# cmavro/GNN-RAG

Measured on NVIDIA H100. Metric: questions/sec (GNN forward+score) on WebQSP-shape subgraphs; agg-kernel HBM GB/s, higher is better.
Workload: dtype f32

## Files before the change

### gnn_rag_b200/csrc/linear_tc.cu

```cuda
#include "wgmma.cuh"

namespace gr {

int g_tc_cluster = 1;
int g_tc_bk = 32;
int g_tc_tma_store = 1;

namespace {

using namespace tc;
constexpr int kThreads = 384;
constexpr int kConsumerWarps = 8;
constexpr int kLaunchRegs = 168, kProducerRegs = 40, kConsumerRegs = 232;
static_assert(128 * kProducerRegs + 256 * kConsumerRegs <= kThreads * kLaunchRegs, "register budget");

__global__ void split_bf16_seg_kernel(const float* __restrict__ W, int64_t ldw, int64_t N, int64_t Kpad,
                                      int seg, int pitch, __nv_bfloat16* __restrict__ hi,
                                      __nv_bfloat16* __restrict__ lo, int64_t ldo) {
  const int64_t total = N * Kpad;
  const int64_t stride = (int64_t)gridDim.x * blockDim.x;
  for (int64_t i = (int64_t)blockIdx.x * blockDim.x + threadIdx.x; i < total; i += stride) {
    const int64_t n = i / Kpad, k = i - n * Kpad;
    const int sidx = (int)(k / pitch), c = (int)(k - (int64_t)sidx * pitch);
    float v = c < seg ? __ldg(W + n * ldw + (int64_t)sidx * seg + c) : 0.f;
    const __nv_bfloat16 h = __float2bfloat16_rn(v);
    hi[n * ldo + k] = h;
    lo[n * ldo + k] = __float2bfloat16_rn(v - __bfloat162float(h));
  }
}

__global__ void split_bf16_kernel(const float* __restrict__ A, int64_t lda, int64_t M, int64_t K,
                                  __nv_bfloat16* __restrict__ hi, __nv_bfloat16* __restrict__ lo,
                                  int64_t ldo, int vec_ok, int vec_st) {
  const int64_t kq = (K + 3) / 4;
  const int64_t total = M * kq;
  const int64_t stride = (int64_t)gridDim.x * blockDim.x;
  for (int64_t i = (int64_t)blockIdx.x * blockDim.x + threadIdx.x; i < total; i += stride) {
    const int64_t m = i / kq, k = (i - m * kq) * 4;
    float v[4] = {0.f, 0.f, 0.f, 0.f};
    const float* src = A + m * lda + k;
    if (vec_ok && k + 3 < K) {
      float4 t = __ldg(reinterpret_cast<const float4*>(src));
      v[0] = t.x; v[1] = t.y; v[2] = t.z; v[3] = t.w;
    } else {
#pragma unroll
      for (int q = 0; q < 4; ++q)
        if (k + q < K) v[q] = __ldg(src + q);
    }
    __nv_bfloat16 h[4], l[4];
#pragma unroll
    for (int q = 0; q < 4; ++q) {
      h[q] = __float2bfloat16_rn(v[q]);
      l[q] = __float2bfloat16_rn(v[q] - __bfloat162float(h[q]));
    }
    __nv_bfloat16* ph = hi + m * ldo + k;
    __nv_bfloat16* pl = lo + m * ldo + k;
    if (vec_st && k + 3 < ldo) {
      *reinterpret_cast<uint2*>(ph) = *reinterpret_cast<uint2*>(h);
      *reinterpret_cast<uint2*>(pl) = *reinterpret_cast<uint2*>(l);
    } else {
#pragma unroll
      for (int q = 0; q < 4; ++q)
        if (k + q < ldo) { ph[q] = h[q]; pl[q] = l[q]; }
    }
  }
}

struct TcParams {
  const float* bias;
  float* C;
  int64_t ldc;
  __nv_bfloat16* c_hi;
  __nv_bfloat16* c_lo;
  int64_t ldc16;
  const float* w_score;
  float* dots;
  int M, N, K, n_pad, n16, stages, num_tiles;
  uint32_t flags;
  int tma_store;
  int kg_T, kg_G, kg_pitch, kg_nkb, kg_one0, kg_one1, kg_nb0;
};

template <int NP, int CS, int BK, bool GROUPED>
__global__ void __launch_bounds__(kThreads, 1)
linear_tc_kernel(const __grid_constant__ CUtensorMap map_a_hi, const __grid_constant__ CUtensorMap map_a_lo,
                 const __grid_constant__ CUtensorMap map_w_hi, const __grid_constant__ CUtensorMap map_w_lo,
                 const __grid_constant__ CUtensorMap map_c, const __grid_constant__ CUtensorMap map_c_hi,
                 const __grid_constant__ CUtensorMap map_c_lo, const TcParams p) {
  extern __shared__ __align__(1024) uint8_t smem_raw[];
  uint8_t* smem = reinterpret_cast<uint8_t*>((reinterpret_cast<uintptr_t>(smem_raw) + 1023) & ~(uintptr_t)1023);
  const int a_bytes = BM * BK * 2;
  constexpr int w_bytes = NP * BK * 2;
  const bool single = (p.flags & GR_LINEAR_BF16_SINGLE) != 0;
  const int w_off = single ? a_bytes : 2 * a_bytes;
  const int stage_bytes = single ? a_bytes + w_bytes : 2 * a_bytes + 2 * w_bytes;
  uint8_t* s_out = smem + (size_t)p.stages * stage_bytes;
  uint64_t* bars = reinterpret_cast<uint64_t*>(s_out + 2 * kStageOutBytes);
  uint64_t* full_bar = bars;
  uint64_t* empty_bar = bars + p.stages;
  float* s_bias = reinterpret_cast<float*>(bars + 2 * p.stages);
  float* s_ws = s_bias + 256;
  for (int i = threadIdx.x; i < 256; i += kThreads) {
    s_bias[i] = (p.bias && i < p.N) ? p.bias[i] : 0.f;
    s_ws[i] = (p.w_score && i < p.N) ? p.w_score[i] : 0.f;
  }

  const int warp = threadIdx.x >> 5, lane = threadIdx.x & 31;
  const int nkb = GROUPED ? p.kg_nkb : (p.K + BK - 1) / BK;
  const int crank = CS > 1 ? (int)cluster_ctarank() : 0;
  const int ncluster = gridDim.x / CS, cid = blockIdx.x / CS;
  const int ngroups = (p.num_tiles + CS - 1) / CS;
  constexpr uint16_t kMask = (uint16_t)((1u << CS) - 1);

  if (threadIdx.x == 0) {
    for (int s = 0; s < p.stages; ++s) {
      mbar_init(&full_bar[s], 1);
      mbar_init(&empty_bar[s], kConsumerWarps * CS);
    }
    asm volatile("fence.mbarrier_init.release.cluster;" ::: "memory");
  }
  __syncthreads();
  if (CS > 1) cluster_sync_all();

  if (warp < 4) {
    asm volatile("setmaxnreg.dec.sync.aligned.u32 %0;" ::"n"(kProducerRegs));
    if (warp == 0 && lane == 0) {
      uint32_t phase = 0;
      int s = 0;
      constexpr int w_rows = NP / CS;
      const int w_slice = w_rows * BK * 2;
      for (int g = cid; g < ngroups; g += ncluster) {
        const int m0 = (g * CS + crank) * BM;
        for (int kb = 0; kb < nkb; ++kb) {
          mbar_wait(&empty_bar[s], phase ^ 1);
          uint8_t* st = smem + (size_t)s * stage_bytes;
          mbar_expect_tx(&full_bar[s], (uint32_t)stage_bytes);
          int a_col = kb * BK;
          if constexpr (GROUPED) {
            if (p.kg_nb0 == 0) {
              const int g = kb / p.kg_T, t = kb - g * p.kg_T, ni = p.kg_T >> 1;
              const int seg = t == 0 ? 0 : 1 + 2 * ((t - 1) % ni) + (t - 1) / ni;
              a_col = seg * p.kg_pitch + g * BK;
            } else {
              const int g = min(kb / p.kg_T, p.kg_G), t = kb - g * p.kg_T;
              a_col = t == 0 ? g * BK : p.kg_nb0 + (kb - g - 1) * BK;
            }
          }
          tma_load_2d(st, &map_a_hi, &full_bar[s], a_col, m0);
          if (!single) tma_load_2d(st + a_bytes, &map_a_lo, &full_bar[s], a_col, m0);
          if (CS == 1) {
            tma_load_2d(st + w_off, &map_w_hi, &full_bar[s], kb * BK, 0);
            if (!single) tma_load_2d(st + w_off + w_bytes, &map_w_lo, &full_bar[s], kb * BK, 0);
          } else {
            tma_load_2d_mc(st + w_off + crank * w_slice, &map_w_hi, &full_bar[s], kb * BK,
                           crank * w_rows, kMask);
            if (!single)
              tma_load_2d_mc(st + w_off + w_bytes + crank * w_slice, &map_w_lo, &full_bar[s], kb * BK,
                             crank * w_rows, kMask);
          }
          if (++s == p.stages) { s = 0; phase ^= 1; }
        }
      }
    }
  } else {
    asm volatile("setmaxnreg.inc.sync.aligned.u32 %0;" ::"n"(kConsumerRegs));
    const int cw = (warp - 4) >> 2, wq = warp & 3;
    const EpiOut e{s_bias, s_ws, (p.flags & GR_LINEAR_RELU) != 0};
    const int r = wq * 16 + (lane >> 2), cq = lane & 3;
    uint8_t* stg = s_out + (size_t)cw * kStageOutBytes;
    const bool issuer = wq == 0 && lane == 0;
    const bool vec_c = p.C && (p.ldc % 2 == 0) && ((reinterpret_cast<uintptr_t>(p.C) & 7) == 0);
    const bool vec_h = p.c_hi && (p.ldc16 % 2 == 0) && ((reinterpret_cast<uintptr_t>(p.c_hi) & 3) == 0) &&
                       ((reinterpret_cast<uintptr_t>(p.c_lo) & 3) == 0);
    uint32_t phase = 0;
    int s = 0;
    for (int g = cid; g < ngroups; g += ncluster) {
      const int tile = g * CS + crank;
      float acc[NP / 2];
#pragma unroll
      for (int i = 0; i < NP / 2; ++i) acc[i] = 0.f;
      int prev = -1;
      for (int kb = 0; kb < nkb; ++kb) {
        mbar_wait(&full_bar[s], phase);
        const uint32_t sa = smem_u32(smem + (size_t)s * stage_bytes);
        const uint32_t a_row = (uint32_t)(cw * WG_M * BK * 2);
        const uint64_t da_hi = make_smem_desc<BK>(sa + a_row), da_lo = make_smem_desc<BK>(sa + a_bytes + a_row);
        const uint64_t dw_hi = make_smem_desc<BK>(sa + w_off), dw_lo = make_smem_desc<BK>(sa + w_off + w_bytes);
        if constexpr (GROUPED) {
          if (kb >= p.kg_one0 && kb < p.kg_one1) mma_kblock<NP, BK, 1, false>(acc, da_hi, da_lo, dw_hi, dw_lo);
          else mma_kblock<NP, BK, BK / MMA_K, false>(acc, da_hi, da_lo, dw_hi, dw_lo);
        } else if (single) {
          mma_kblock<NP, BK, BK / MMA_K, true>(acc, da_hi, da_lo, dw_hi, dw_lo);
        } else {
          mma_kblock<NP, BK, BK / MMA_K, false>(acc, da_hi, da_lo, dw_hi, dw_lo);
        }
        wgmma_wait<1>();
        if (prev >= 0 && lane == 0) release_slot<CS>(&empty_bar[prev]);
        prev = s;
        if (++s == p.stages) { s = 0; phase ^= 1; }
      }
      wgmma_wait<0>();
      if (prev >= 0 && lane == 0) release_slot<CS>(&empty_bar[prev]);

      const int64_t row0 = (int64_t)tile * BM + cw * WG_M + r;
      float dot0 = 0.f, dot1 = 0.f;
#pragma unroll
      for (int q = 0; q < NP / 16; ++q) {
        const int c0 = 16 * q;
        if (c0 >= p.n_pad) continue;
        float v[8];
        epi_values(acc, q, cq, e, v, dot0, dot1);
        if (p.tma_store) {
          epi_store_tma(v, stg, r, cq, issuer, 1 + cw, &map_c, &map_c_hi, &map_c_lo, p.C != nullptr,
                        p.c_hi != nullptr, c0, tile * BM + cw * WG_M);
          continue;
        }
#pragma unroll
        for (int b = 0; b < 2; ++b) {
          const int col = c0 + 8 * b + 2 * cq;
#pragma unroll
          for (int hr = 0; hr < 2; ++hr) {
            const int64_t row = row0 + 8 * hr;
            if (row >= p.M) continue;
            const float x0 = v[4 * b + 2 * hr], x1 = v[4 * b + 2 * hr + 1];
            if (p.C) {
              float* c = p.C + row * p.ldc + col;
              if (vec_c && col + 1 < p.N) {
                *reinterpret_cast<float2*>(c) = make_float2(x0, x1);
              } else {
                if (col < p.N) c[0] = x0;
                if (col + 1 < p.N) c[1] = x1;
              }
            }
            if (p.c_hi) {
              uint32_t lo;
              const uint32_t hi = split_hi_lo(x0, x1, lo);
              unsigned short* ph = reinterpret_cast<unsigned short*>(p.c_hi + row * p.ldc16 + col);
              unsigned short* pl = reinterpret_cast<unsigned short*>(p.c_lo + row * p.ldc16 + col);
              if (vec_h && col + 1 < p.n16) {
                *reinterpret_cast<uint32_t*>(ph) = hi;
                *reinterpret_cast<uint32_t*>(pl) = lo;
              } else {
                if (col < p.n16) { ph[0] = (unsigned short)(hi & 0xFFFF); pl[0] = (unsigned short)(lo & 0xFFFF); }
                if (col + 1 < p.n16) { ph[1] = (unsigned short)(hi >> 16); pl[1] = (unsigned short)(lo >> 16); }
              }
            }
          }
        }
      }
      epi_dots(dot0, dot1, p.dots, row0, p.M, cq);
    }
    if (p.tma_store && issuer) asm volatile("cp.async.bulk.wait_group 0;" ::: "memory");
  }
  __syncthreads();
  if (CS > 1) cluster_sync_all();
}

struct TcPlan {
  int64_t kp;
  int n_pad, np, stages, bk;
  size_t a_plane_bytes, w_plane_bytes, total_bytes, w_only_bytes, smem_bytes;
  bool ok;
};

TcPlan plan_tc(int64_t M, int64_t N, int64_t K, bool single = false) {
  TcPlan t{};
  const int BK = g_tc_bk == 64 ? 64 : 32;
  t.ok = (N >= 8 && N <= 256 && K >= 8 && M >= 1);
  t.kp = (K + 7) / 8 * 8;
  t.n_pad = (int)((N + 15) / 16 * 16);
  t.np = t.n_pad <= 64 ? 64 : t.n_pad <= 128 ? 128 : t.n_pad <= 208 ? 208 : 256;
  const size_t stage = (single ? 1 : 2) * ((size_t)BM * BK * 2 + (size_t)t.np * BK * 2);
  int stages = (int)((227 * 1024 - 1024 - 2048 - 128 - 2 * kStageOutBytes) / stage);
  t.stages = stages > 8 ? 8 : stages;
  if (t.stages < 2) t.ok = false;
  t.bk = BK;
  t.smem_bytes = (size_t)t.stages * stage + 1024  + 2 * t.stages * 8 + 2 * 256 * 4 + 2 * kStageOutBytes;
  t.a_plane_bytes = align_up((size_t)M * t.kp * 2, 256);
  t.w_plane_bytes = align_up((size_t)N * t.kp * 2, 256);
  t.total_bytes = 2 * t.a_plane_bytes + 2 * t.w_plane_bytes;
  t.w_only_bytes = 2 * t.w_plane_bytes;
  return t;
}


int split_launch(const float* A, int64_t lda, int64_t M, int64_t K, __nv_bfloat16* hi, __nv_bfloat16* lo,
                 int64_t ldo, cudaStream_t stream) {
  int va = (lda % 4 == 0) && ((reinterpret_cast<uintptr_t>(A) & 15) == 0);
  int64_t work = M * ((K + 3) / 4);
  int grid = (int)std::min<int64_t>(ceil_div(work, 256), 32LL * sm_count());
  int vs = (ldo % 4 == 0) && ((reinterpret_cast<uintptr_t>(hi) & 7) == 0) &&
           ((reinterpret_cast<uintptr_t>(lo) & 7) == 0);
  split_bf16_kernel<<<grid, 256, 0, stream>>>(A, lda, M, K, hi, lo, ldo, va, vs);
  GR_CHECK_LAUNCH();
  return GR_OK;
}

template <int NP, int CS, int BK, bool GROUPED = false>
int launch_tc_cs(const CUtensorMap& m_a_hi, const CUtensorMap& m_a_lo, const CUtensorMap& m_w_hi,
                 const CUtensorMap& m_w_lo, const CUtensorMap& m_c, const CUtensorMap& m_c_hi,
                 const CUtensorMap& m_c_lo, const TcPlan& t, const TcParams& p, cudaStream_t stream) {
  const int ngroups = (p.num_tiles + CS - 1) / CS;
  const int nclusters = std::max(1, std::min(ngroups, sm_count() / CS));
  return launch_cluster<linear_tc_kernel<NP, CS, BK, GROUPED>>("gr_linear_tc", kLaunchRegs, CS, nclusters * CS, kThreads,
                                                               t.smem_bytes, stream, m_a_hi, m_a_lo, m_w_hi, m_w_lo,
                                                               m_c, m_c_hi, m_c_lo, p);
}

template <int NP>
int launch_tc_np(const CUtensorMap* const (&m)[7], int cs, const TcPlan& t, const TcParams& p, cudaStream_t stream) {
  if (p.kg_T) {
    if (cs == 2) return launch_tc_cs<NP, 2, 32, true>(*m[0], *m[1], *m[2], *m[3], *m[4], *m[5], *m[6], t, p, stream);
    return launch_tc_cs<NP, 1, 32, true>(*m[0], *m[1], *m[2], *m[3], *m[4], *m[5], *m[6], t, p, stream);
  }
  if (t.bk == 64) {
    if (cs == 2) return launch_tc_cs<NP, 2, 64>(*m[0], *m[1], *m[2], *m[3], *m[4], *m[5], *m[6], t, p, stream);
    return launch_tc_cs<NP, 1, 64>(*m[0], *m[1], *m[2], *m[3], *m[4], *m[5], *m[6], t, p, stream);
  }
  if (cs == 2) return launch_tc_cs<NP, 2, 32>(*m[0], *m[1], *m[2], *m[3], *m[4], *m[5], *m[6], t, p, stream);
  return launch_tc_cs<NP, 1, 32>(*m[0], *m[1], *m[2], *m[3], *m[4], *m[5], *m[6], t, p, stream);
}

int launch_tc(const __nv_bfloat16* a_hi, const __nv_bfloat16* a_lo, int64_t lda16,
              const __nv_bfloat16* w_hi, const __nv_bfloat16* w_lo, int64_t ldw16, const TcPlan& t,
              TcParams p, cudaStream_t stream) {
  p.n_pad = t.n_pad; p.stages = t.stages;
  p.num_tiles = (int)ceil_div(p.M, BM);
  int cs = (g_tc_cluster >= 2 && (t.np / 2) % 8 == 0 && p.num_tiles >= 2) ? 2 : 1;
  CUtensorMap m_a_hi, m_a_lo, m_w_hi, m_w_lo;
  const int64_t w_cols = p.kg_T ? ldw16 : p.K;
  const int64_t a_cols = p.kg_nb0 ? p.kg_nb0 + (int64_t)(p.kg_T - 1) * p.kg_pitch : p.K;
  if (!make_tmap(&m_a_hi, a_hi, p.M, a_cols, lda16, BM, t.bk) || !make_tmap(&m_a_lo, a_lo, p.M, a_cols, lda16, BM, t.bk) ||
      !make_tmap(&m_w_hi, w_hi, p.N, w_cols, ldw16, t.np / cs, t.bk) ||
      !make_tmap(&m_w_lo, w_lo, p.N, w_cols, ldw16, t.np / cs, t.bk)) {
    set_error("gr_linear_tc: cuTensorMapEncodeTiled failed (pointers must be 16-byte aligned, row strides "
              "multiples of 8 elements)");
    return GR_ERR_CUDA;
  }
  p.n16 = (int)std::min<int64_t>((p.N + 15) / 16 * 16, p.ldc16);
  CUtensorMap m_c, m_c_hi, m_c_lo;
  memset(&m_c, 0, sizeof(m_c)); memset(&m_c_hi, 0, sizeof(m_c_hi)); memset(&m_c_lo, 0, sizeof(m_c_lo));
  bool ok = g_tc_tma_store != 0;
  if (ok && p.C) ok = p.N % 4 == 0 && make_out_tmap(&m_c, p.C, p.M, p.N, p.ldc, 4);
  if (ok && p.c_hi) ok = make_out_tmap(&m_c_hi, p.c_hi, p.M, p.n16, p.ldc16, 2) &&
                         make_out_tmap(&m_c_lo, p.c_lo, p.M, p.n16, p.ldc16, 2);
  p.tma_store = ok ? 1 : 0;
  const CUtensorMap* m[7] = {&m_a_hi, &m_a_lo, &m_w_hi, &m_w_lo, &m_c, &m_c_hi, &m_c_lo};
  switch (t.np) {
    case 64: return launch_tc_np<64>(m, cs, t, p, stream);
    case 128: return launch_tc_np<128>(m, cs, t, p, stream);
    case 208: return launch_tc_np<208>(m, cs, t, p, stream);
    default: return launch_tc_np<256>(m, cs, t, p, stream);
  }
}

}

bool linear_tc_supported(int64_t M, int64_t N, int64_t K) {
  return plan_tc(M, N, K).ok && get_encode_fn() != nullptr;
}

}

extern "C" size_t gr_linear_tc_workspace_bytes(int64_t M, int64_t N, int64_t K) {
  if (M <= 0 || N <= 0 || K <= 0) return 0;
  return gr::plan_tc(M, N, K).total_bytes;
}

extern "C" size_t gr_linear_tc_planes_workspace_bytes(int64_t N, int64_t K) {
  if (N <= 0 || K <= 0) return 0;
  return gr::plan_tc(1, N, K).w_only_bytes;
}

extern "C" int gr_split_bf16(const float* A, int64_t lda, int64_t M, int64_t K, void* hi, void* lo,
                             int64_t ld_out, void* stream_) {
  using namespace gr;
  GR_CHECK_ARG(A && hi && lo, "null pointer");
  GR_CHECK_ARG(M > 0 && K > 0 && lda >= K && ld_out >= K && ld_out % 8 == 0, "bad shape / ld_out % 8 != 0");
  return split_launch(A, lda, M, K, reinterpret_cast<__nv_bfloat16*>(hi), reinterpret_cast<__nv_bfloat16*>(lo),
                      ld_out, reinterpret_cast<cudaStream_t>(stream_));
}

extern "C" int gr_linear_tc(const float* A, int64_t lda, const float* W, int64_t ldw, const float* bias,
                            float* C, int64_t ldc, int64_t M, int64_t N, int64_t K, uint32_t flags,
                            void* workspace, size_t workspace_bytes, void* stream_) {
  using namespace gr;
  cudaStream_t stream = reinterpret_cast<cudaStream_t>(stream_);
  GR_CHECK_ARG(A && W && C && workspace, "null pointer");
  GR_CHECK_ARG(M > 0 && N > 0 && K > 0, "M, N, K must be positive");
  GR_CHECK_ARG(lda >= K && ldw >= K && ldc >= N, "leading dimension smaller than row length");
  GR_CHECK_ARG(M < (int64_t)0x7fffffff - BM, "M exceeds int32 range");
  TcPlan t = plan_tc(M, N, K);
  if (!t.ok) {
    set_error("gr_linear_tc: unsupported shape M=%lld N=%lld K=%lld (need 8 <= N <= 256, K >= 8)",
              (long long)M, (long long)N, (long long)K);
    return GR_ERR_UNSUPPORTED;
  }
  if (int rc = check_workspace(__func__, workspace, workspace_bytes, t.total_bytes)) return rc;
  if ((reinterpret_cast<uintptr_t>(workspace) & 255) != 0) {
    set_error("gr_linear_tc: workspace must be 256-byte aligned");
    return GR_ERR_INVALID_ARG;
  }
  char* ws = reinterpret_cast<char*>(workspace);
  __nv_bfloat16* a_hi = reinterpret_cast<__nv_bfloat16*>(ws);
  __nv_bfloat16* a_lo = reinterpret_cast<__nv_bfloat16*>(ws + t.a_plane_bytes);
  __nv_bfloat16* w_hi = reinterpret_cast<__nv_bfloat16*>(ws + 2 * t.a_plane_bytes);
  __nv_bfloat16* w_lo = reinterpret_cast<__nv_bfloat16*>(ws + 2 * t.a_plane_bytes + t.w_plane_bytes);
  int rc = split_launch(A, lda, M, K, a_hi, a_lo, t.kp, stream);
  if (rc != GR_OK) return rc;
  rc = split_launch(W, ldw, N, K, w_hi, w_lo, t.kp, stream);
  if (rc != GR_OK) return rc;
  TcParams p{};
  p.bias = bias; p.C = C; p.ldc = ldc;
  p.M = (int)M; p.N = (int)N; p.K = (int)K; p.flags = flags;
  return launch_tc(a_hi, a_lo, t.kp, w_hi, w_lo, t.kp, t, p, stream);
}

extern "C" int gr_linear_tc_planes(const void* A_hi, const void* A_lo, int64_t lda16, const float* W,
                                   int64_t ldw, const float* bias, float* C, int64_t ldc, void* C_hi,
                                   void* C_lo, int64_t ldc16, const float* w_score, float* dots, int64_t M,
                                   int64_t N, int64_t K, int64_t k_seg, int64_t k_seg_pitch, uint32_t flags,
                                   void* workspace, size_t workspace_bytes, void* stream_) {
  using namespace gr;
  cudaStream_t stream = reinterpret_cast<cudaStream_t>(stream_);
  GR_CHECK_ARG(A_hi && (A_lo || (flags & GR_LINEAR_BF16_SINGLE)) && W && workspace, "null pointer");
  GR_CHECK_ARG(C || C_hi, "no output requested");
  GR_CHECK_ARG(M > 0 && N > 0 && K > 0, "M, N, K must be positive");
  const bool grouped = (flags & GR_LINEAR_K_GROUPED) != 0;
  const bool korder = (flags & GR_LINEAR_K_ORDER_PLANES) != 0;
  GR_CHECK_ARG(!korder || grouped, "GR_LINEAR_K_ORDER_PLANES modifies GR_LINEAR_K_GROUPED and needs it");
  if (grouped) {
    GR_CHECK_ARG(k_seg > 0 && k_seg_pitch >= k_seg && k_seg_pitch % 16 == 0,
                 "GR_LINEAR_K_GROUPED needs segmented K: k_seg > 0 and k_seg_pitch >= k_seg, a multiple of 16");
    GR_CHECK_ARG(K % k_seg_pitch == 0 && (K / k_seg_pitch) % 2 == 1,
                 "GR_LINEAR_K_GROUPED needs an odd number of segments (2 I + 1)");
    GR_CHECK_ARG(g_tc_bk != 64, "GR_LINEAR_K_GROUPED needs 32-column k-blocks (tc_bk = 32)");
    GR_CHECK_ARG(!(flags & GR_LINEAR_BF16_SINGLE), "GR_LINEAR_K_GROUPED does not combine with GR_LINEAR_BF16_SINGLE");
  }
  const bool segmented = grouped || (k_seg > 0 && k_seg_pitch > k_seg);
  GR_CHECK_ARG(lda16 >= K && lda16 % 8 == 0, "lda16 must be >= K and a multiple of 8");
  GR_CHECK_ARG(!segmented || K % k_seg_pitch == 0, "K must be a multiple of k_seg_pitch");
  GR_CHECK_ARG(ldw >= (segmented ? K / k_seg_pitch * k_seg : K), "ldw smaller than the weight row length");
  GR_CHECK_ARG(!C || ldc >= N, "ldc smaller than N");
  GR_CHECK_ARG(!C_hi || (C_lo && ldc16 >= N), "C_lo missing or ldc16 smaller than N");
  GR_CHECK_ARG(!dots || w_score, "dots requested without w_score");
  GR_CHECK_ARG(M < (int64_t)0x7fffffff - BM, "M exceeds int32 range");
  TcPlan t = plan_tc(M, N, K, (flags & GR_LINEAR_BF16_SINGLE) != 0);
  if (!t.ok) {
    set_error("gr_linear_tc_planes: unsupported shape M=%lld N=%lld K=%lld", (long long)M, (long long)N,
              (long long)K);
    return GR_ERR_UNSUPPORTED;
  }
  const int num_ins = grouped ? (int)(K / k_seg_pitch / 2) : 0;
  const GroupedK gk = grouped ? plan_grouped_k(k_seg_pitch, num_ins, N, korder) : GroupedK{};
// ... 46 lines not shown
```

### gnn_rag_b200/csrc/wgmma.cuh

```cuda
#pragma once
#include <cuda.h>
#include <cuda_bf16.h>

#include "common.cuh"

namespace gr {
namespace tc {

constexpr int BM = 128;
constexpr int WG_M = 64;
constexpr int MMA_K = 16;

struct GroupedK {
  int G, ksteps_last, nkb;
  int64_t kp;
  size_t w_plane_bytes;
};
GroupedK plan_grouped_k(int64_t pitch, int I, int64_t N_out, bool packed = false);
int grouped_w_split(const float* W, int64_t ldw, int64_t N_out, int D, int I, const GroupedK& k, __nv_bfloat16* hi,
                    __nv_bfloat16* lo, cudaStream_t stream);

typedef CUresult (*EncodeTiledFn)(CUtensorMap*, CUtensorMapDataType, cuuint32_t, void*, const cuuint64_t*,
                                  const cuuint64_t*, const cuuint32_t*, const cuuint32_t*,
                                  CUtensorMapInterleave, CUtensorMapSwizzle, CUtensorMapL2promotion,
                                  CUtensorMapFloatOOBfill);

inline EncodeTiledFn get_encode_fn() {
  static EncodeTiledFn fn = nullptr;
  static bool tried = false;
  if (!tried) {
    tried = true;
    void* p = nullptr;
    cudaDriverEntryPointQueryResult q;
    if (cudaGetDriverEntryPoint("cuTensorMapEncodeTiled", &p, cudaEnableDefault, &q) == cudaSuccess &&
        q == cudaDriverEntryPointSuccess)
      fn = reinterpret_cast<EncodeTiledFn>(p);
  }
  return fn;
}

inline bool make_tmap(CUtensorMap* m, const void* base, int64_t rows, int64_t cols, int64_t ld, int box_rows,
               int bk) {
  EncodeTiledFn fn = get_encode_fn();
  if (!fn) return false;
  cuuint64_t dims[2] = {(cuuint64_t)cols, (cuuint64_t)rows};
  cuuint64_t strides[1] = {(cuuint64_t)ld * 2};
  cuuint32_t box[2] = {(cuuint32_t)bk, (cuuint32_t)box_rows};
  cuuint32_t estr[2] = {1, 1};
  CUresult r = fn(m, CU_TENSOR_MAP_DATA_TYPE_BFLOAT16, 2, const_cast<void*>(base), dims, strides, box, estr,
                  CU_TENSOR_MAP_INTERLEAVE_NONE,
                  bk == 64 ? CU_TENSOR_MAP_SWIZZLE_128B : CU_TENSOR_MAP_SWIZZLE_64B,
                  CU_TENSOR_MAP_L2_PROMOTION_L2_256B, CU_TENSOR_MAP_FLOAT_OOB_FILL_NONE);
  return r == CUDA_SUCCESS;
}

inline bool make_out_tmap(CUtensorMap* m, const void* base, int64_t rows, int64_t cols, int64_t ld, int elem_bytes) {
  EncodeTiledFn fn = get_encode_fn();
  if (!fn) return false;
  if ((reinterpret_cast<uintptr_t>(base) & 15) != 0 || (ld * elem_bytes) % 16 != 0) return false;
  cuuint64_t dims[2] = {(cuuint64_t)cols, (cuuint64_t)rows};
  cuuint64_t strides[1] = {(cuuint64_t)ld * elem_bytes};
  cuuint32_t box[2] = {16u, (cuuint32_t)WG_M};
  cuuint32_t estr[2] = {1, 1};
  CUresult r = fn(m, elem_bytes == 4 ? CU_TENSOR_MAP_DATA_TYPE_FLOAT32 : CU_TENSOR_MAP_DATA_TYPE_BFLOAT16, 2,
                  const_cast<void*>(base), dims, strides, box, estr, CU_TENSOR_MAP_INTERLEAVE_NONE,
                  CU_TENSOR_MAP_SWIZZLE_NONE, CU_TENSOR_MAP_L2_PROMOTION_NONE,
                  CU_TENSOR_MAP_FLOAT_OOB_FILL_NONE);
  return r == CUDA_SUCCESS;
}

__device__ __forceinline__ uint32_t smem_u32(const void* p) {
  return (uint32_t)__cvta_generic_to_shared(p);
}
__device__ __forceinline__ void mbar_init(uint64_t* bar, uint32_t count) {
  asm volatile("mbarrier.init.shared::cta.b64 [%0], %1;" ::"r"(smem_u32(bar)), "r"(count));
}
__device__ __forceinline__ void mbar_expect_tx(uint64_t* bar, uint32_t bytes) {
  asm volatile("mbarrier.arrive.expect_tx.shared::cta.b64 _, [%0], %1;" ::"r"(smem_u32(bar)), "r"(bytes)
               : "memory");
}
__device__ __forceinline__ void mbar_wait(uint64_t* bar, uint32_t parity) {
  uint32_t ok = 0;
  while (!ok) {
    asm volatile(
        "{\n\t.reg .pred p;\n\t"
        "mbarrier.try_wait.parity.shared::cta.b64 p, [%1], %2;\n\t"
        "selp.u32 %0, 1, 0, p;\n\t}"
        : "=r"(ok)
        : "r"(smem_u32(bar)), "r"(parity)
        : "memory");
  }
}
__device__ __forceinline__ void mbar_arrive(uint64_t* bar) {
  asm volatile("mbarrier.arrive.shared::cta.b64 _, [%0];" ::"r"(smem_u32(bar)) : "memory");
}
__device__ __forceinline__ void mbar_arrive_cluster(uint64_t* bar, uint32_t rank) {
  uint32_t remote;
  asm volatile("mapa.shared::cluster.u32 %0, %1, %2;" : "=r"(remote) : "r"(smem_u32(bar)), "r"(rank));
  asm volatile("mbarrier.arrive.release.cluster.shared::cluster.b64 _, [%0];" ::"r"(remote) : "memory");
}
template <int CS>
__device__ __forceinline__ void release_slot(uint64_t* bar) {
  if (CS == 1) {
    mbar_arrive(bar);
  } else {
#pragma unroll
    for (int r = 0; r < CS; ++r) mbar_arrive_cluster(bar, (uint32_t)r);
  }
}
__device__ __forceinline__ void tma_load_2d(void* dst, const CUtensorMap* map, uint64_t* bar, int c0,
                                            int c1) {
  asm volatile(
      "cp.async.bulk.tensor.2d.shared::cluster.global.tile.mbarrier::complete_tx::bytes"
      " [%0], [%1, {%3, %4}], [%2];" ::"r"(smem_u32(dst)),
      "l"(reinterpret_cast<uint64_t>(map)), "r"(smem_u32(bar)), "r"(c0), "r"(c1)
      : "memory");
}
__device__ __forceinline__ void tma_load_2d_mc(void* dst, const CUtensorMap* map, uint64_t* bar, int c0,
                                               int c1, uint16_t mask) {
  asm volatile(
      "cp.async.bulk.tensor.2d.shared::cluster.global.tile.mbarrier::complete_tx::bytes.multicast::cluster"
      " [%0], [%1, {%4, %5}], [%2], %3;" ::"r"(smem_u32(dst)),
      "l"(reinterpret_cast<uint64_t>(map)), "r"(smem_u32(bar)), "h"(mask), "r"(c0), "r"(c1)
      : "memory");
}
__device__ __forceinline__ void tma_store_2d(const CUtensorMap* map, const void* src, int c0, int c1) {
  asm volatile("cp.async.bulk.tensor.2d.global.shared::cta.bulk_group [%0, {%2, %3}], [%1];" ::"l"(
                   reinterpret_cast<uint64_t>(map)),
               "r"(smem_u32(src)), "r"(c0), "r"(c1)
               : "memory");
}
__device__ __forceinline__ void named_bar_sync(int id, int nthreads) {
  asm volatile("bar.sync %0, %1;" ::"r"(id), "r"(nthreads) : "memory");
}
__device__ __forceinline__ void cluster_sync_all() {
  asm volatile("barrier.cluster.arrive.release.aligned;" ::: "memory");
  asm volatile("barrier.cluster.wait.acquire.aligned;" ::: "memory");
}
__device__ __forceinline__ uint32_t cluster_ctarank() {
  uint32_t r;
  asm volatile("mov.u32 %0, %%cluster_ctarank;" : "=r"(r));
  return r;
}

template <int BK>
__device__ __forceinline__ uint64_t make_smem_desc(uint32_t saddr) {
  uint64_t d = 0;
  d |= (uint64_t)((saddr >> 4) & 0x3FFF);
  d |= (uint64_t)1 << 16;
  d |= (uint64_t)((8 * BK * 2) >> 4) << 32;
  d |= (uint64_t)(BK == 64 ? 1 : 2) << 62;
  return d;
}

__device__ __forceinline__ void wgmma_fence() { asm volatile("wgmma.fence.sync.aligned;" ::: "memory"); }
__device__ __forceinline__ void wgmma_commit() { asm volatile("wgmma.commit_group.sync.aligned;" ::: "memory"); }
template <int N>
__device__ __forceinline__ void wgmma_wait() {
  asm volatile("wgmma.wait_group.sync.aligned %0;" ::"n"(N) : "memory");
}
template <int R>
__device__ __forceinline__ void acc_fence(float (&d)[R]) {
#pragma unroll
  for (int i = 0; i < R; ++i) asm volatile("" : "+f"(d[i])::"memory");
}

#define GR_ACC8(i) "+f"(d[OFF + (i)]), "+f"(d[OFF + (i) + 1]), "+f"(d[OFF + (i) + 2]), "+f"(d[OFF + (i) + 3]), \
                   "+f"(d[OFF + (i) + 4]), "+f"(d[OFF + (i) + 5]), "+f"(d[OFF + (i) + 6]), "+f"(d[OFF + (i) + 7])
#define GR_ACC32(i) GR_ACC8(i), GR_ACC8((i) + 8), GR_ACC8((i) + 16), GR_ACC8((i) + 24)
#define GR_REGS8 "%0, %1, %2, %3, %4, %5, %6, %7"
#define GR_REGS16 GR_REGS8 ", %8, %9, %10, %11, %12, %13, %14, %15"
#define GR_REGS32 GR_REGS16 ", %16, %17, %18, %19, %20, %21, %22, %23, %24, %25, %26, %27, %28, %29, %30, %31"
#define GR_REGS64 GR_REGS32 ", %32, %33, %34, %35, %36, %37, %38, %39, %40, %41, %42, %43, %44, %45, %46, %47, %48, " \
                  "%49, %50, %51, %52, %53, %54, %55, %56, %57, %58, %59, %60, %61, %62, %63"
#define GR_REGS104 GR_REGS64 ", %64, %65, %66, %67, %68, %69, %70, %71, %72, %73, %74, %75, %76, %77, %78, %79, " \
                   "%80, %81, %82, %83, %84, %85, %86, %87, %88, %89, %90, %91, %92, %93, %94, %95, %96, %97, %98, " \
                   "%99, %100, %101, %102, %103"
#define GR_REGS128 GR_REGS104 ", %104, %105, %106, %107, %108, %109, %110, %111, %112, %113, %114, %115, %116, " \
                   "%117, %118, %119, %120, %121, %122, %123, %124, %125, %126, %127"
#define GR_WGMMA(N, REGS, RA, RB, ...)                                                                   \
  asm volatile("{\n\t.reg .pred p;\n\tsetp.ne.b32 p, 1, 0;\n\t"                                          \
               "wgmma.mma_async.sync.aligned.m64n" #N "k16.f32.bf16.bf16 {" REGS "}, %" #RA ", %" #RB  \
               ", p, 1, 1, 0, 0;\n\t}"                                                                   \
               : __VA_ARGS__                                                                             \
               : "l"(a), "l"(b))
template <int N, int OFF, int R>
__device__ __forceinline__ void wgmma_bf16(float (&d)[R], uint64_t a, uint64_t b) {
  static_assert(OFF + N / 2 <= R, "accumulator range");
  if constexpr (N == 16) {
    GR_WGMMA(16, GR_REGS8, 8, 9, GR_ACC8(0));
// ... 47 lines not shown
}

struct EpiOut {
  const float* bias;
  const float* w_score;
  bool relu;
};

template <int R>
__device__ __forceinline__ void epi_values(const float (&a)[R], int q, int cq, const EpiOut& e, float (&v)[8],
                                           float& dot0, float& dot1) {
#pragma unroll
  for (int b = 0; b < 2; ++b) {
    const int col = 16 * q + 8 * b + 2 * cq;
    const float2 bb = *reinterpret_cast<const float2*>(e.bias + col);
    const float2 ww = *reinterpret_cast<const float2*>(e.w_score + col);
#pragma unroll
    for (int i = 0; i < 4; ++i) {
      float x = a[8 * q + 4 * b + i] + ((i & 1) ? bb.y : bb.x);
      if (e.relu) x = fmaxf(x, 0.f);
      v[4 * b + i] = x;
    }
    dot0 = fmaf(v[4 * b + 0], ww.x, dot0); dot0 = fmaf(v[4 * b + 1], ww.y, dot0);
    dot1 = fmaf(v[4 * b + 2], ww.x, dot1); dot1 = fmaf(v[4 * b + 3], ww.y, dot1);
  }
}

__device__ __forceinline__ uint32_t split_hi_lo(float x0, float x1, uint32_t& lo) {
  const __nv_bfloat162 h2 = __floats2bfloat162_rn(x0, x1);
  const float2 hf = __bfloat1622float2(h2);
  const __nv_bfloat162 l2 = __floats2bfloat162_rn(x0 - hf.x, x1 - hf.y);
  lo = *reinterpret_cast<const uint32_t*>(&l2);
  return *reinterpret_cast<const uint32_t*>(&h2);
}

constexpr int kStageOutBytes = WG_M * 16 * 4 + 2 * WG_M * 16 * 2;
__device__ __forceinline__ void epi_store_tma(const float (&v)[8], uint8_t* stg, int r, int cq, bool issuer,
                                              int bar_id, const CUtensorMap* map_c, const CUtensorMap* map_hi,
                                              const CUtensorMap* map_lo, bool has_c, bool has_planes, int c0, int m0) {
  if (issuer) asm volatile("cp.async.bulk.wait_group.read 0;" ::: "memory");
  named_bar_sync(bar_id, 128);
  float* s_c = reinterpret_cast<float*>(stg);
  uint32_t* s_h = reinterpret_cast<uint32_t*>(stg + WG_M * 16 * 4);
  uint32_t* s_l = reinterpret_cast<uint32_t*>(stg + WG_M * 16 * 4 + WG_M * 16 * 2);
#pragma unroll
  for (int b = 0; b < 2; ++b) {
    const int col = 8 * b + 2 * cq;
#pragma unroll
    for (int hr = 0; hr < 2; ++hr) {
      const int row = r + 8 * hr;
      const float x0 = v[4 * b + 2 * hr], x1 = v[4 * b + 2 * hr + 1];
      if (has_c) *reinterpret_cast<float2*>(s_c + row * 16 + col) = make_float2(x0, x1);
      if (has_planes) {
        uint32_t lo;
        const uint32_t hi = split_hi_lo(x0, x1, lo);
        s_h[row * 8 + col / 2] = hi;
        s_l[row * 8 + col / 2] = lo;
      }
    }
  }
  asm volatile("fence.proxy.async.shared::cta;" ::: "memory");
  named_bar_sync(bar_id, 128);
  if (issuer) {
    if (has_c) tma_store_2d(map_c, stg, c0, m0);
    if (has_planes) {
      tma_store_2d(map_hi, stg + WG_M * 16 * 4, c0, m0);
      tma_store_2d(map_lo, stg + WG_M * 16 * 4 + WG_M * 16 * 2, c0, m0);
    }
    asm volatile("cp.async.bulk.commit_group;" ::: "memory");
  }
}

__device__ __forceinline__ void epi_dots(float dot0, float dot1, float* dots, int64_t row0, int64_t M, int cq) {
  dot0 += __shfl_xor_sync(0xffffffffu, dot0, 1);
  dot0 += __shfl_xor_sync(0xffffffffu, dot0, 2);
  dot1 += __shfl_xor_sync(0xffffffffu, dot1, 1);
  dot1 += __shfl_xor_sync(0xffffffffu, dot1, 2);
  if (dots && cq == 0) {
    if (row0 < M) { dots[row0] = dot0; dots[M + row0] = 0.f; }
    if (row0 + 8 < M) { dots[row0 + 8] = dot1; dots[M + row0 + 8] = 0.f; }
  }
}

template <auto Kernel, typename... Args>
int launch_cluster(const char* fn, int launch_regs, int cs, int grid, int threads, size_t smem, cudaStream_t stream,
                   const Args&... args) {
  if (int rc = opt_in_smem<Kernel>(fn, 227 * 1024)) return rc;
  static int num_regs = 0;
  if (num_regs == 0) {
    cudaFuncAttributes fa{};
    GR_CHECK_CUDA_AS(fn, cudaFuncGetAttributes(&fa, Kernel));
    num_regs = fa.numRegs;
  }
  if (num_regs != launch_regs) {
    set_error("%s: kernel was compiled with %d registers per thread, the warpgroup budget needs %d", fn, num_regs,
              launch_regs);
    return GR_ERR_UNSUPPORTED;
  }
  cudaLaunchConfig_t cfg{};
  cfg.gridDim = dim3((unsigned)grid);
  cfg.blockDim = dim3((unsigned)threads);
  cfg.dynamicSmemBytes = smem;
  cfg.stream = stream;
  cudaLaunchAttribute attr[1];
  attr[0].id = cudaLaunchAttributeClusterDimension;
  attr[0].val.clusterDim.x = cs;
  attr[0].val.clusterDim.y = 1;
  attr[0].val.clusterDim.z = 1;
  cfg.attrs = attr;
  cfg.numAttrs = 1;
  GR_CHECK_CUDA_AS(fn, cudaLaunchKernelEx(&cfg, Kernel, args...));
  return GR_OK;
}

}
}
```

### include/gnnrag_b200.h

```cpp
#ifndef GNNRAG_B200_H_
#define GNNRAG_B200_H_

#include <stddef.h>
#include <stdint.h>

#ifdef __cplusplus
extern "C" {
#endif

#define GR_ABI_VERSION 1

typedef enum gr_status {
  GR_OK = 0,
  GR_ERR_INVALID_ARG = -1,
  GR_ERR_CUDA = -2,
  GR_ERR_WORKSPACE = -3,
  GR_ERR_UNSUPPORTED = -4
} gr_status;

#define GR_LINEAR_RELU 1u
#define GR_LINEAR_EXACT_FP32 2u
#define GR_LINEAR_BF16_SINGLE 8u
#define GR_LINEAR_W_PRESPLIT 4u

#define GR_LINEAR_K_GROUPED 16u
#define GR_LINEAR_K_ORDER_PLANES 32u

int gr_abi_version(void);
const char* gr_last_error(void);
int gr_set_option(const char* name, int64_t value);
static inline int64_t gr_pad4(int64_t n) { return (n + 3) & ~(int64_t)3; }

size_t gr_csr_build_workspace_bytes(int64_t F, int64_t Nt);
int gr_csr_build(const void* heads, const void* rels, const void* tails, int idx_bytes,
                 int64_t F, int64_t Nt, int64_t num_rel_rows,
                 int32_t* rowptr_t, int32_t* src_t, int32_t* rel_t, int32_t* fact_t,
                 int32_t* rowptr_h, int32_t* src_h, int32_t* rel_h, int32_t* fact_h,
                 int32_t* status, const int32_t* nfacts, void* workspace, size_t workspace_bytes, void* stream);

int gr_gather_f32(const float* in, const int32_t* fact, float* out, int64_t F, void* stream);

int gr_linear(const float* A, int64_t lda, const float* W, int64_t ldw, const float* bias,
              const float* addend, int64_t ld_addend, int64_t addend_rows,
              float* C, int64_t ldc, int64_t M, int64_t N, int64_t K, uint32_t flags, void* stream);

size_t gr_linear_tc_workspace_bytes(int64_t M, int64_t N, int64_t K);
int gr_linear_tc(const float* A, int64_t lda, const float* W, int64_t ldw, const float* bias,
                 float* C, int64_t ldc, int64_t M, int64_t N, int64_t K, uint32_t flags,
                 void* workspace, size_t workspace_bytes, void* stream);
size_t gr_linear_tc_planes_workspace_bytes(int64_t N, int64_t K);
int gr_linear_tc_planes(const void* A_hi, const void* A_lo, int64_t lda16, const float* W, int64_t ldw,
                        const float* bias, float* C, int64_t ldc, void* C_hi, void* C_lo, int64_t ldc16,
                        const float* w_score, float* dots, int64_t M, int64_t N, int64_t K,
                        int64_t k_seg, int64_t k_seg_pitch,
                        uint32_t flags, void* workspace, size_t workspace_bytes, void* stream);
int gr_split_bf16(const float* A, int64_t lda, int64_t M, int64_t K, void* hi, void* lo, int64_t ld_out,
                  void* stream);

int gr_aggregate(const int32_t* rowptr, const int32_t* src, const int32_t* rel, const float* w,
                 const float* prior, const float* table, const float* ins,
                 float* out, int64_t out_row_stride, int64_t out_col0, int64_t seg_stride,
                 float* possible, int B, int N, int D, int I, int64_t F, void* stream);

int gr_aggregate_backward(const int32_t* rowptr, const int32_t* src, const int32_t* rel, const float* w,
                          const float* prior, const float* table, const float* ins, const float* grad_out,
                          int64_t grad_row_stride, int64_t grad_col0, int64_t seg_stride, float* grad_table,
                          float* grad_ins, float* grad_prior, int B, int N, int D, int I, int64_t F, void* stream);

int gr_aggregate_dual(const int32_t* rowptr_t, const int32_t* src_t, const int32_t* rel_t,
                      const float* w_t, const int32_t* rowptr_h, const int32_t* src_h,
                      const int32_t* rel_h, const float* w_h, const float* prior,
                      const float* table_fwd, const float* table_inv, const float* ins,
                      float* out, int64_t out_row_stride, int64_t out_col0, int64_t seg_pitch,
                      void* out_hi, void* out_lo, int64_t ld_planes,
                      int B, int N, int D, int I, int64_t F, void* stream);

int gr_pad_table256(const float* table, int64_t ldt, int64_t rows, int D, float* pn, void* stream);
int gr_aggregate_dual_abs_supported(int N, int D, int64_t seg_pitch, int64_t R1);
int gr_aggregate_dual_abs(const int32_t* rowptr_t, const int32_t* src_t, const int32_t* rel_t, const float* w_t,
                         const int32_t* rowptr_h, const int32_t* src_h, const int32_t* rel_h, const float* w_h,
                         const float* prior, const float* pn_fwd, const float* pn_inv, int64_t table_rows,
                         const float* ins, void* out_hi, void* out_lo, int64_t ld_planes, int64_t out_col0,
                         int64_t seg_pitch, int B, int N, int D, int I, int64_t F, int32_t* tile_counter, void* stream);
#define GR_AGG_K_ORDER 1u
int gr_aggregate_dual_abs_ex(const int32_t* rowptr_t, const int32_t* src_t, const int32_t* rel_t, const float* w_t,
                             const int32_t* rowptr_h, const int32_t* src_h, const int32_t* rel_h, const float* w_h,
                             const float* prior, const float* pn_fwd, const float* pn_inv, int64_t table_rows,
                             const float* ins, void* out_hi, void* out_lo, int64_t ld_planes, int64_t out_col0,
                             int64_t seg_pitch, int B, int N, int D, int I, int64_t F, int32_t* tile_counter,
                             uint32_t flags, void* stream);

int gr_fused_profile_read(unsigned long long* out, int n);
int gr_fused_layer_supported(int64_t N_nodes, int64_t D, int64_t seg_pitch, int I, int64_t N_out);
size_t gr_fused_layer_workspace_bytes(int64_t D, int64_t seg_pitch, int I, int64_t N_out);
size_t gr_fused_ell_bytes(int B, int N_nodes, int64_t F);
int gr_fused_ell_build(const int32_t* rowptr_t, const int32_t* src_t, const int32_t* rel_t, const float* w_t,
                       const int32_t* rowptr_h, const int32_t* src_h, const int32_t* rel_h, const float* w_h,
                       int B, int N_nodes, int64_t F, void* ell, size_t ell_bytes, void* stream);
int gr_fused_layer(const int32_t* rowptr_t, const int32_t* src_t, const int32_t* rel_t, const float* w_t,
                   const int32_t* rowptr_h, const int32_t* src_h, const int32_t* rel_h, const float* w_h,
                   const float* prior, const float* pn_fwd, const float* pn_inv, const float* ins,
                   const void* h_hi, const void* h_lo, int64_t ldh16, int64_t seg_pitch, const float* W,
                   int64_t ldw, const float* bias, float* C, int64_t ldc, void* C_hi, void* C_lo,
                   int64_t ldc16, const float* w_score, float* dots, int B, int N_nodes, int D, int I,
                   int64_t N_out, int64_t F, uint32_t flags, void* workspace, size_t workspace_bytes,
                   void* ell, size_t ell_bytes, void* stream);

int gr_debug_store_probe(void* hi, void* lo, int64_t Nt, int64_t ld, int col_start, int ncols, int mode,
                         void* stream);

int gr_type_layer(const int32_t* rowptr_t, const int32_t* rel_t, const float* w_t,
                  const int32_t* rowptr_h, const int32_t* rel_h, const float* w_h,
                  const float* table, float* out, int64_t out_row_stride,
                  void* out_hi, void* out_lo, int64_t ld_planes,
                  int B, int N, int D, int64_t F, void* stream);

size_t gr_graft_stage_workspace_bytes(int64_t B, int64_t max_fact);
int gr_graft_stage(const int64_t* e2f_b, const int64_t* e2f_f, const int64_t* e2f_e, int64_t F_e2f,
                   const int64_t* f2e_b, const int64_t* f2e_e, const int64_t* f2e_f, int64_t F_f2e,
                   const int64_t* kb_fact_rel, int B, int N, int64_t max_fact, int64_t R1, int32_t* heads,
                   int32_t* rels, int32_t* tails, int32_t* slot_of, int32_t* nfacts, int32_t* status,
                   const int32_t* live, void* workspace, size_t workspace_bytes, void* stream);
int gr_graft_attention(const float* qh, const float* qmask, int Q, const float* rel, int64_t ldr, int64_t R1,
                       const int64_t* kb_fact_rel, int B, int64_t max_fact, int D, const int32_t* rowptr_h,
                       const int32_t* fact_h, const int32_t* slot_of, int N, float* W, float* Wt, float* E,
                       int32_t* status, void* stream);
int gr_graft_aggregate(const int32_t* rowptr_t, const int32_t* src_t, const int32_t* rel_t, const int32_t* fact_t,
                       const int32_t* slot_of, const float* Wt, const float* E, const float* prior,
                       const float* self_tab, int64_t ld_self, const float* head_tab, int64_t ld_head,
                       const float* q2e, double lambda, float* sum_out, int64_t ld_sum, void* out_hi, void* out_lo,
                       int64_t ld_planes, int64_t col_sum, int64_t col_indeg, int64_t col_q2e, float* indeg_out,
                       float* prior_next, int B, int N, int D, void* stream);

int gr_graft_dropout_mask(const int64_t* seed, double p, int64_t S, int D, uint8_t* mask, void* stream);
int gr_graft_aggregate_train(const int32_t* rowptr_t, const int32_t* src_t, const int32_t* rel_t,
                             const int32_t* fact_t, const int32_t* slot_of, const float* s, const float* self_tab,
                             int64_t ld_self, const float* head_tab, int64_t ld_head, const int64_t* seed, double p,
                             float* sum_out, int64_t ld_sum, int B, int N, int D, void* stream);
// ... 258 lines not shown
```

Measured before the change: 12890.

## Auto-select 2-CTA clusters and size persistent grid by occupancy query

Result: faster. 13060, median of 6 (+1.3%).

```diff
diff --git a/gnn_rag_b200/csrc/linear_tc.cu b/gnn_rag_b200/csrc/linear_tc.cu
--- a/gnn_rag_b200/csrc/linear_tc.cu
+++ b/gnn_rag_b200/csrc/linear_tc.cu
@@ -2,9 +2,23 @@
 
 namespace gr {
 
-int g_tc_cluster = 1;
+int g_tc_cluster = 0;
 int g_tc_bk = 32;
 int g_tc_tma_store = 1;
+
+int tc_cluster_grid(int64_t num_tiles, int cs, int max_active_clusters) {
+  const int64_t ngroups = (num_tiles + cs - 1) / cs;
+  return (int)std::max<int64_t>(1, std::min<int64_t>(ngroups, max_active_clusters));
+}
+
+int tc_cluster_size(int np, int64_t num_tiles, bool k_order) {
+  const bool pair_ok = (np / 2) % 8 == 0 && num_tiles >= 2;
+  if (g_tc_cluster == 1 || !pair_ok) return 1;
+  if (g_tc_cluster >= 2) return 2;
+  return k_order && np == 208 && num_tiles >= 4 * (int64_t)sm_count() ? 2 : 1;
+}
+
+int g_tc_last_launch[3] = {0, 0, 0};
 
 namespace {
 
@@ -131,10 +145,15 @@
       const int w_slice = w_rows * BK * 2;
       for (int g = cid; g < ngroups; g += ncluster) {
         const int m0 = (g * CS + crank) * BM;
+#ifdef GR_LINEAR_TC_DIAG_W_FIRST_TILE
+        const bool load_w = g == cid;
+#else
+        constexpr bool load_w = true;
+#endif
         for (int kb = 0; kb < nkb; ++kb) {
           mbar_wait(&empty_bar[s], phase ^ 1);
           uint8_t* st = smem + (size_t)s * stage_bytes;
-          mbar_expect_tx(&full_bar[s], (uint32_t)stage_bytes);
+          mbar_expect_tx(&full_bar[s], (uint32_t)(load_w ? stage_bytes : w_off));
           int a_col = kb * BK;
           if constexpr (GROUPED) {
             if (p.kg_nb0 == 0) {
@@ -148,10 +167,10 @@
           }
           tma_load_2d(st, &map_a_hi, &full_bar[s], a_col, m0);
           if (!single) tma_load_2d(st + a_bytes, &map_a_lo, &full_bar[s], a_col, m0);
-          if (CS == 1) {
+          if (load_w && CS == 1) {
             tma_load_2d(st + w_off, &map_w_hi, &full_bar[s], kb * BK, 0);
             if (!single) tma_load_2d(st + w_off + w_bytes, &map_w_lo, &full_bar[s], kb * BK, 0);
-          } else {
+          } else if (load_w) {
             tma_load_2d_mc(st + w_off + crank * w_slice, &map_w_hi, &full_bar[s], kb * BK,
                            crank * w_rows, kMask);
             if (!single)
@@ -195,12 +214,12 @@
           mma_kblock<NP, BK, BK / MMA_K, false>(acc, da_hi, da_lo, dw_hi, dw_lo);
         }
         wgmma_wait<1>();
-        if (prev >= 0 && lane == 0) release_slot<CS>(&empty_bar[prev]);
+        if (prev >= 0 && lane == 0) release_slot<CS, false>(&empty_bar[prev]);
         prev = s;
         if (++s == p.stages) { s = 0; phase ^= 1; }
       }
       wgmma_wait<0>();
-      if (prev >= 0 && lane == 0) release_slot<CS>(&empty_bar[prev]);
+      if (prev >= 0 && lane == 0) release_slot<CS, false>(&empty_bar[prev]);
 
       const int64_t row0 = (int64_t)tile * BM + cw * WG_M + r;
       float dot0 = 0.f, dot1 = 0.f;
@@ -300,11 +319,13 @@
 int launch_tc_cs(const CUtensorMap& m_a_hi, const CUtensorMap& m_a_lo, const CUtensorMap& m_w_hi,
                  const CUtensorMap& m_w_lo, const CUtensorMap& m_c, const CUtensorMap& m_c_hi,
                  const CUtensorMap& m_c_lo, const TcPlan& t, const TcParams& p, cudaStream_t stream) {
-  const int ngroups = (p.num_tiles + CS - 1) / CS;
-  const int nclusters = std::max(1, std::min(ngroups, sm_count() / CS));
-  return launch_cluster<linear_tc_kernel<NP, CS, BK, GROUPED>>("gr_linear_tc", kLaunchRegs, CS, nclusters * CS, kThreads,
-                                                               t.smem_bytes, stream, m_a_hi, m_a_lo, m_w_hi, m_w_lo,
-                                                               m_c, m_c_hi, m_c_lo, p);
+  constexpr auto kernel = linear_tc_kernel<NP, CS, BK, GROUPED>;
+  int max_active = 0;
+  if (int rc = max_active_clusters<kernel>("gr_linear_tc", CS, kThreads, t.smem_bytes, &max_active)) return rc;
+  const int nclusters = tc_cluster_grid(p.num_tiles, CS, max_active);
+  g_tc_last_launch[0] = CS; g_tc_last_launch[1] = nclusters; g_tc_last_launch[2] = max_active;
+  return launch_cluster<kernel>("gr_linear_tc", kLaunchRegs, CS, nclusters * CS, kThreads, t.smem_bytes, stream,
+                                m_a_hi, m_a_lo, m_w_hi, m_w_lo, m_c, m_c_hi, m_c_lo, p);
 }
 
 template <int NP>
@@ -326,7 +347,7 @@
               TcParams p, cudaStream_t stream) {
   p.n_pad = t.n_pad; p.stages = t.stages;
   p.num_tiles = (int)ceil_div(p.M, BM);
-  int cs = (g_tc_cluster >= 2 && (t.np / 2) % 8 == 0 && p.num_tiles >= 2) ? 2 : 1;
+  const int cs = tc_cluster_size(t.np, p.num_tiles, p.kg_nb0 > 0);
   CUtensorMap m_a_hi, m_a_lo, m_w_hi, m_w_lo;
   const int64_t w_cols = p.kg_T ? ldw16 : p.K;
   const int64_t a_cols = p.kg_nb0 ? p.kg_nb0 + (int64_t)(p.kg_T - 1) * p.kg_pitch : p.K;
@@ -370,6 +391,18 @@
 extern "C" size_t gr_linear_tc_planes_workspace_bytes(int64_t N, int64_t K) {
   if (N <= 0 || K <= 0) return 0;
   return gr::plan_tc(1, N, K).w_only_bytes;
+}
+
+extern "C" int gr_linear_tc_cluster_grid(int64_t num_tiles, int cluster, int max_active_clusters) {
+  if (num_tiles < 1 || cluster < 1 || max_active_clusters < 1) return 0;
+  return gr::tc_cluster_grid(num_tiles, cluster, max_active_clusters);
+}
+
+extern "C" int gr_linear_tc_last_launch(int* cluster, int* clusters, int* max_active_clusters) {
+  if (cluster) *cluster = gr::g_tc_last_launch[0];
+  if (clusters) *clusters = gr::g_tc_last_launch[1];
+  if (max_active_clusters) *max_active_clusters = gr::g_tc_last_launch[2];
+  return GR_OK;
 }
 
 extern "C" int gr_split_bf16(const float* A, int64_t lda, int64_t M, int64_t K, void* hi, void* lo,
diff --git a/gnn_rag_b200/csrc/wgmma.cuh b/gnn_rag_b200/csrc/wgmma.cuh
--- a/gnn_rag_b200/csrc/wgmma.cuh
+++ b/gnn_rag_b200/csrc/wgmma.cuh
@@ -94,18 +94,22 @@
 __device__ __forceinline__ void mbar_arrive(uint64_t* bar) {
   asm volatile("mbarrier.arrive.shared::cta.b64 _, [%0];" ::"r"(smem_u32(bar)) : "memory");
 }
+template <bool CLUSTER_SCOPE = true>
 __device__ __forceinline__ void mbar_arrive_cluster(uint64_t* bar, uint32_t rank) {
   uint32_t remote;
   asm volatile("mapa.shared::cluster.u32 %0, %1, %2;" : "=r"(remote) : "r"(smem_u32(bar)), "r"(rank));
-  asm volatile("mbarrier.arrive.release.cluster.shared::cluster.b64 _, [%0];" ::"r"(remote) : "memory");
-}
-template <int CS>
+  if constexpr (CLUSTER_SCOPE)
+    asm volatile("mbarrier.arrive.release.cluster.shared::cluster.b64 _, [%0];" ::"r"(remote) : "memory");
+  else
+    asm volatile("mbarrier.arrive.shared::cluster.b64 _, [%0];" ::"r"(remote) : "memory");
+}
+template <int CS, bool CLUSTER_SCOPE = true>
 __device__ __forceinline__ void release_slot(uint64_t* bar) {
   if (CS == 1) {
     mbar_arrive(bar);
   } else {
 #pragma unroll
-    for (int r = 0; r < CS; ++r) mbar_arrive_cluster(bar, (uint32_t)r);
+    for (int r = 0; r < CS; ++r) mbar_arrive_cluster<CLUSTER_SCOPE>(bar, (uint32_t)r);
   }
 }
 __device__ __forceinline__ void tma_load_2d(void* dst, const CUtensorMap* map, uint64_t* bar, int c0,
@@ -319,6 +323,43 @@
   }
 }
 
+template <auto Kernel>
+int max_active_clusters(const char* fn, int cs, int threads, size_t smem, int* out) {
+  struct Entry { size_t smem; int n; };
+  static Entry cache[64][4] = {};
+  int dev = 0;
+  GR_CHECK_CUDA_AS(fn, cudaGetDevice(&dev));
+  Entry* row = dev >= 0 && dev < 64 ? cache[dev] : nullptr;
+  if (row)
+    for (int i = 0; i < 4; ++i)
+      if (row[i].n > 0 && row[i].smem == smem) { *out = row[i].n; return GR_OK; }
+  if (int rc = opt_in_smem<Kernel>(fn, 227 * 1024)) return rc;
+  cudaLaunchConfig_t cfg{};
+  cfg.gridDim = dim3((unsigned)(cs * sm_count()));
+  cfg.blockDim = dim3((unsigned)threads);
+  cfg.dynamicSmemBytes = smem;
+  cudaLaunchAttribute attr[1];
+  attr[0].id = cudaLaunchAttributeClusterDimension;
+  attr[0].val.clusterDim.x = cs;
+  attr[0].val.clusterDim.y = 1;
+  attr[0].val.clusterDim.z = 1;
+  cfg.attrs = attr;
+  cfg.numAttrs = 1;
+  int n = 0;
+  GR_CHECK_CUDA_AS(fn, cudaOccupancyMaxActiveClusters(&n, Kernel, &cfg));
+  if (n < 1) {
+    set_error("%s: no cluster of %d CTAs with %zu bytes of shared memory fits on the device", fn, cs, smem);
+    return GR_ERR_UNSUPPORTED;
+  }
+  if (row) {
+    int i = 0;
+    while (i < 3 && row[i].n > 0) ++i;
+    row[i] = Entry{smem, n};
+  }
+  *out = n;
+  return GR_OK;
+}
+
 template <auto Kernel, typename... Args>
 int launch_cluster(const char* fn, int launch_regs, int cs, int grid, int threads, size_t smem, cudaStream_t stream,
                    const Args&... args) {
diff --git a/include/gnnrag_b200.h b/include/gnnrag_b200.h
--- a/include/gnnrag_b200.h
+++ b/include/gnnrag_b200.h
@@ -54,6 +54,8 @@
                         const float* w_score, float* dots, int64_t M, int64_t N, int64_t K,
                         int64_t k_seg, int64_t k_seg_pitch,
                         uint32_t flags, void* workspace, size_t workspace_bytes, void* stream);
+int gr_linear_tc_cluster_grid(int64_t num_tiles, int cluster, int max_active_clusters);
+int gr_linear_tc_last_launch(int* cluster, int* clusters, int* max_active_clusters);
 int gr_split_bf16(const float* A, int64_t lda, int64_t M, int64_t K, void* hi, void* lo, int64_t ld_out,
                   void* stream);
 
```
